# claymore666/openhush

Hardware: AMD Instinct MI355X
Metric: audio-sec/sec (xRT) large-v3 greedy, 30s chunks, 1/2/4/8 MI355X (higher is better)
Workload: dtype bf16; 1 GPU; large-v3 dims, steps of batch=32 x 30 s windows per GPU, greedy, 100 tokens/window (EOT suppressed), procedural weights seed 1234, every window a distinct synthetic recording, PCM resident in HBM; schedule LANES 4x3: 12 steps (384 windows) in flight per GPU - per lane ONE front-end pass and ONE decode batch of 96 rows, 4 decodes side by side on 64 CUs each; concurrent_sub_batches=1

## Files before the change

include/ohw.h:

```cpp
#ifndef OHW_H
#define OHW_H

#include <stddef.h>
#include <stdint.h>

#ifdef __cplusplus
extern "C" {
#endif

#define OHW_ABI_VERSION 2

enum {
  OHW_OK = 0,
  OHW_E_MODEL_NOT_FOUND = -3001,
  OHW_E_LOAD_FAILED = -3002,
  OHW_E_TRANSCRIBE = -3003,
  OHW_E_NO_GPU = -3004,
  OHW_E_OOM = -3005,
  OHW_E_INVALID_ARG = -3006,
  OHW_E_VALIDATION = -3007
};

enum { OHW_DTYPE_AUTO = -1, OHW_DTYPE_BF16 = 0, OHW_DTYPE_F16 = 1 };

// ... 463 lines not shown
typedef struct {
  ohw_dbg_beam_io base;
  const float* plog;
  float* plog_next;
  float* fin_plog;
  float* nosp_prob;
} ohw_dbg_beam_io_ex;
int ohw_dbg_beam_step_ex(ohw_state* st, const ohw_sample_params* p, const ohw_dbg_beam_io_ex* io);

typedef struct {
  int32_t K, W, stride, max_tokens;
  const int32_t* fin_cnt;
  const int32_t* fin_len;
  const float* fin_sum;
  const int32_t* fin_tok;
  const float* fin_plog;
  const int32_t* n_cur;
  const int32_t* tokens;
  const float* plog;
  const float* beam_sum;
  int32_t* out_tokens;
  float* out_logprobs;
  int32_t* n_tokens;
  float* sum_logprob;
  int32_t* ended_by_eot;
  int32_t* n_finished;
} ohw_beam_finish_io;
int ohw_dbg_beam_finish(ohw_state* st, const ohw_beam_finish_io* io);
int ohw_beam_finish_host(const ohw_beam_finish_io* io);

enum { OHW_DEPI_QKV = 0, OHW_DEPI_BIAS_T, OHW_DEPI_BIAS_GELU_T, OHW_DEPI_BIAS_RESID, OHW_DEPI_LOGITS };
enum { OHW_DG_FORM_PLAIN = 0, OHW_DG_FORM_LN, OHW_DG_FORM_PN };
enum { OHW_DG_SHAPE_1x1 = 0, OHW_DG_SHAPE_2x1, OHW_DG_SHAPE_1x2, OHW_DG_SHAPE_2x2, OHW_DG_SHAPE_4x2, OHW_DG_SHAPE_1x6,
       OHW_DG_SHAPE_4x6, OHW_DG_SHAPE_5x6 };
typedef struct {
  int32_t dtype, epilogue, form;
  int32_t M, N, K, n_new;
  int64_t ld_out;
  int32_t cu_budget, ksplit;
  const float* w;
  const float* bias;
  const float* gamma;
  const float* beta;
  const void* x;
  const float* stat_in;
  void* out;
  float* slab;
  int64_t slab_bytes;
  uint32_t* ticket;
  void* x16_out;
  float* stat_out;
  void* k_cache;
  void* v_cache;
  const int32_t* n_past;
  int32_t d_model, n_head, n_ctx;
  int32_t* shape_out;
} ohw_dbg_dec_gemm_io;
int ohw_dbg_dec_gemm(const ohw_dbg_dec_gemm_io* io, void* stream);
int ohw_dbg_embed(int dtype, const float* emb, int n_vocab, const float* pos, int n_pos, const int32_t* tok_host,
                  const int32_t* n_past_host, float* x, void* x16, float* stat, int M, int n_new, int d, void* stream);
int ohw_dbg_layernorm(int dtype, const float* x, const float* gamma, const float* beta, void* y, int64_t rows, int d, int tiled,
                      void* stream);

enum { OHW_EG_KERNEL_AUTO = 0, OHW_EG_KERNEL_K128, OHW_EG_KERNEL_SMALL, OHW_EG_KERNEL_K256 };
typedef struct {
  int32_t dtype, epilogue, kernel;
  int32_t conv_cin;
  int64_t M, N, K;
  int64_t lda, a_batch_stride, rows_per_batch;
  int64_t ldc, c_batch_stride;
  int32_t d_model, n_head, t_len, batch, batch_offset;
  const int32_t* c_row_map;
  const void* a;
  int64_t a_elems;
  const float* w;
  const float* bias;
  const float* pos;
  void* out;
  int64_t out_elems;
} ohw_dbg_enc_gemm_io;
int ohw_dbg_enc_gemm(const ohw_dbg_enc_gemm_io* io, void* stream);

#ifdef __cplusplus
}
#endif
#endif
```

openhush_amd/csrc/decode.hip:

```cpp
#include <algorithm>
#include <type_traits>

#include "kernels.hpp"

namespace ohw {

#ifdef OHW_TRACE
__device__ unsigned long long ohw_trace_buf[1 << 18];
__device__ unsigned ohw_trace_n;
__device__ __forceinline__ void trace_mark(unsigned id, unsigned stage) {
  const unsigned nb = gridDim.x * gridDim.y * gridDim.z, bi = (blockIdx.z * gridDim.y + blockIdx.y) * gridDim.x + blockIdx.x;
  __builtin_amdgcn_sched_barrier(0);
  if (threadIdx.x == 0 && (bi == 0 || bi == nb - 1 || bi == nb / 2)) {
    const unsigned k = atomicAdd(&ohw_trace_n, 1u);
    if (k < (1u << 18)) ohw_trace_buf[k] = ((unsigned long long)wall_clock64() << 16) | (id << 8) | (stage << 2) | (bi == 0 ? 0 : bi == nb - 1 ? 1 : 2);
  }
}
#define TRACE(id, stage) trace_mark(id, stage)
#else
#define TRACE(id, stage)
#endif

template <typename T>
__global__ void embed_kernel(const T* __restrict__ emb, const float* __restrict__ pos, const int32_t* __restrict__ tok,
// ... 493 lines not shown
        else
          self_attn_row<T, false, true>((const T*)p.out, (const T*)p.k_cache, (const T*)p.v_cache, n_keys, m, m, head, p.n_head, p.n_ctx,
                                        nullptr, (T*)p.attn_out, qs, ps, lane, (unsigned)p.kv_bytes);
      }
    }
  }
  TRACE(16 + EPI * 2 + (LN ? 1 : 0), 3);
}

template <typename T, int EPI, bool LN, int NT, int MT>
static int dec_gemm_launch(const DecGemmParams& p, hipStream_t s) {
  const int n_tiles = (p.N + 15) / 16;
  dim3 grid((n_tiles + NT - 1) / NT, (p.M + 16 * MT - 1) / (16 * MT), p.ksplit > 1 ? p.ksplit : 1);
  const size_t smem = (size_t)DG_WAVES * NT * 2 * 64 * 16 + (LN ? (size_t)16 * MT * (p.K * 2 + 16) : 256);
  if (LN) ensure_dynamic_lds((const void*)dec_gemm_kernel<T, EPI, LN, NT, MT>, 160 * 1024);
  hipLaunchKernelGGL((dec_gemm_kernel<T, EPI, LN, NT, MT>), grid, dim3(DG_THREADS), smem, s, p);
  return NT == 4 ? DG_SHAPE_4x2 : NT == 2 ? (MT == 1 ? DG_SHAPE_2x1 : DG_SHAPE_2x2) : (MT == 1 ? DG_SHAPE_1x1 : DG_SHAPE_1x2);
}

template <typename T>
__global__ __launch_bounds__(128) void dec_ln_rows_kernel(const float* __restrict__ x, T* __restrict__ y, int M, int K) {
  const int row = threadIdx.x >> 4, sub = threadIdx.x & 15;
  const int m = blockIdx.x * 8 + row;
  const int mc = m < M ? m : M - 1;
  dec_ln_row<T, 16>(x + (int64_t)mc * K, K, sub, [&](int c, u32x2 w2) {
    if (m >= M) w2 = (u32x2){0u, 0u};
    *(u32x2*)(y + act_tiled_offset(m, c, K)) = w2;
  });
}

template <typename T, int EPI, int NTW, int MTP, int PASSES, int G>
__global__ __launch_bounds__(DG_THREADS, 2) void dec_gemm_rows_kernel(DecGemmParams p) {
  constexpr bool HOLD = EPI != DEPI_BIAS_RESID;
  static_assert(HOLD ? (EPI == DEPI_QKV || EPI == DEPI_BIAS_GELU_T) : (NTW == 1 && PASSES == 1), "rows form");
  using Ops = TypeOps<T>;
  using vec8 = typename Ops::vec8;
  extern __shared__ __attribute__((aligned(16))) unsigned char dg_smem[];
  f32x4* part = (f32x4*)dg_smem;
  const int tid = threadIdx.x, lane = tid & 63, wave = tid >> 6;
  const int nt0 = blockIdx.x * NTW;
  const int n_tiles = (p.N + 15) / 16;
  const int kblocks = p.K / 32;
  TRACE(16 + EPI * 2, 0);
  constexpr int NE = (NTW * MTP * 256 + DG_THREADS - 1) / DG_THREADS;
  [[maybe_unused]] float resid_old[NE];
  if constexpr (!HOLD) {
#pragma unroll
    for (int i = 0; i < NE; ++i) {
      const int idx = tid + DG_THREADS * i, ll = (idx >> 2) & 63;
      const int m = (blockIdx.y * MTP + (idx >> 8)) * 16 + (ll & 15), n = nt0 * 16 + 4 * (ll >> 4) + (idx & 3);
      resid_old[i] = (idx < MTP * 256 && m < p.M && n < p.N) ? ((const float*)p.out)[(int64_t)m * p.ld_out + n] : 0.f;
    }
  }
  const vec8* wt[NTW];
#pragma unroll
  for (int t = 0; t < NTW; ++t) {
    int nt = nt0 + t;
    if (nt > n_tiles - 1) nt = n_tiles - 1;
    wt[t] = (const vec8*)p.w + (int64_t)nt * kblocks * 64 + lane;
  }
  constexpr int UL = DG_LN_MAXK / 32 / DG_WAVES;
  [[maybe_unused]] vec8 whold[HOLD ? NTW : 1][UL];
  if constexpr (HOLD) {
#pragma unroll
    for (int u = 0; u < UL; ++u) {
      int kk = wave + DG_WAVES * u;
      if (kk > kblocks - 1) kk = kblocks - 1;
#pragma unroll
      for (int t = 0; t < NTW; ++t) whold[t][u] = __builtin_nontemporal_load(&wt[t][(int64_t)kk * 64]);
    }
  }

#pragma unroll 1
  for (int pass = 0; pass < PASSES; ++pass) {
    const int mt0 = (blockIdx.y * PASSES + pass) * MTP;
    if (mt0 * 16 >= p.M) break;
    [[maybe_unused]] const T* x0 = (const T*)p.x + ((int64_t)mt0 * kblocks * 64 + lane) * 8;
    bool ok[MTP];
#pragma unroll
    for (int q = 0; q < MTP; ++q) ok[q] = (mt0 + q) * 16 + (lane & 15) < p.M;
    f32x4 acc[NTW][MTP];
#pragma unroll
    for (int t = 0; t < NTW; ++t)
#pragma unroll
      for (int q = 0; q < MTP; ++q) acc[t][q] = (f32x4){0.f, 0.f, 0.f, 0.f};

    if constexpr (HOLD) {
      typedef __attribute__((ext_vector_type(4))) unsigned u32v4;
      const int mt_last = (p.M - 1) >> 4;
      u32v4 a32[MTP][UL];
#pragma unroll
      for (int q = 0; q < MTP; ++q) {
        const int mq = mt0 + q < mt_last ? mt0 + q : mt_last;
        const T* xq = (const T*)p.x + ((int64_t)mq * kblocks * 64 + lane) * 8;
#pragma unroll
        for (int u = 0; u < UL; ++u) {
          const int kk = wave + DG_WAVES * u;
          a32[q][u] = *(const u32v4*)(xq + (int64_t)(kk < kblocks ? kk : 0) * 512);
        }
      }
      vec8 a[MTP][UL];
#pragma unroll
      for (int q = 0; q < MTP; ++q)
#pragma unroll
        for (int u = 0; u < UL; ++u) {
          const unsigned keep = (ok[q] && wave + DG_WAVES * u < kblocks) ? 0xffffffffu : 0u;
          a[q][u] = __builtin_bit_cast(vec8, a32[q][u] & keep);
        }
      __builtin_amdgcn_sched_barrier(0);
#pragma unroll
      for (int u = 0; u < UL; ++u)
#pragma unroll
        for (int t = 0; t < NTW; ++t)
#pragma unroll
          for (int q = 0; q < MTP; ++q) acc[t][q] = Ops::mfma16(whold[t][u], a[q][u], acc[t][q]);
    } else {
      auto run = [&](auto ucount, int kb) {
        constexpr int U = decltype(ucount)::value;
        constexpr int GG = U < G ? U : G;
        static_assert(U % GG == 0, "U");
        vec8 w[U];
#pragma unroll
        for (int u = 0; u < U; ++u) w[u] = __builtin_nontemporal_load(&wt[0][(int64_t)(kb + DG_WAVES * u) * 64]);
#pragma unroll
        for (int g = 0; g < U; g += GG) {
          vec8 a[MTP][GG];
#pragma unroll
          for (int q = 0; q < MTP; ++q) {
#pragma unroll
            for (int u = 0; u < GG; ++u)
#pragma unroll
// ... 10 lines not shown
            for (int q = 0; q < MTP; ++q) acc[0][q] = Ops::mfma16(w[g + u], a[q][u], acc[0][q]);
        }
      };
      int kb = wave;
      for (; kb + DG_WAVES * 19 < kblocks; kb += DG_WAVES * 20) run(std::integral_constant<int, 20>{}, kb);
      for (; kb + DG_WAVES * 3 < kblocks; kb += DG_WAVES * 4) run(std::integral_constant<int, 4>{}, kb);
      for (; kb < kblocks; kb += DG_WAVES) run(std::integral_constant<int, 1>{}, kb);
    }

    TRACE(16 + EPI * 2, 2);
    int etid = tid;
    if constexpr (HOLD) {
      __builtin_amdgcn_sched_barrier(0);
      asm volatile("" : "+v"(etid));
    }
    if (pass > 0) __syncthreads();
#pragma unroll
    for (int t = 0; t < NTW; ++t)
#pragma unroll
      for (int q = 0; q < MTP; ++q) part[((wave * NTW + t) * MTP + q) * 64 + lane] = acc[t][q];
    __syncthreads();
    const float* pp = (const float*)part;
#pragma unroll
    for (int i = 0; i < NE; ++i) {
      const int idx = etid + DG_THREADS * i;
      if (idx >= NTW * MTP * 256) continue;
      const int t = idx / (MTP * 256), q = (idx % (MTP * 256)) >> 8, ll = (idx >> 2) & 63, reg = idx & 3;
      float v = 0.f;
#pragma unroll
      for (int w = 0; w < DG_WAVES; ++w) v += pp[(((w * NTW + t) * MTP + q) * 64 + ll) * 4 + reg];
      const int m = (mt0 + q) * 16 + (ll & 15), n = (nt0 + t) * 16 + 4 * (ll >> 4) + reg;
      if (m >= p.M || n >= p.N || nt0 + t >= n_tiles) continue;
      if (p.bias) v += p.bias[n];
      if constexpr (HOLD) dec_gemm_store16<T, EPI>(p, m, n, v);
      else ((float*)p.out)[(int64_t)m * p.ld_out + n] = resid_old[i] + v;
    }
  }
  TRACE(16 + EPI * 2, 3);
}

template <typename T, int EPI, int NTW, int MTP, int PASSES, int G>
static void dec_gemm_rows_launch(const DecGemmParams& p, hipStream_t s) {
  const int n_tiles = (p.N + 15) / 16, mt = (p.M + 15) / 16;
  const size_t smem = (size_t)DG_WAVES * NTW * MTP * 64 * 16;
  if (smem > 64 * 1024) ensure_dynamic_lds((const void*)dec_gemm_rows_kernel<T, EPI, NTW, MTP, PASSES, G>, 160 * 1024);
  hipLaunchKernelGGL((dec_gemm_rows_kernel<T, EPI, NTW, MTP, PASSES, G>), dim3((n_tiles + NTW - 1) / NTW, (mt + MTP * PASSES - 1) / (MTP * PASSES)),
                     dim3(DG_THREADS), smem, s, p);
}

template <typename T, int EPI, int NTW>
static int dec_gemm_lnrows_launch(const DecGemmParams& p, hipStream_t s) {
  const int mt = (p.M + 15) / 16;
  hipLaunchKernelGGL((dec_ln_rows_kernel<T>), dim3(2 * mt), dim3(128), 0, s, (const float*)p.x, (T*)p.ln_rows, p.M, p.K);
  DecGemmParams q = p;
  q.x = p.ln_rows; q.ln = 0;
  dec_gemm_rows_launch<T, EPI, NTW, 3, 2, 5>(q, s);
  return NTW == 4 ? DG_SHAPE_4x6 : DG_SHAPE_5x6;
}

template <typename T, int EPI, bool LN>
static int dec_gemm_pick(const DecGemmParams& p, hipStream_t s) {
  const int n_tiles = (p.N + 15) / 16;
  static const int logits_nt = getenv("OHW_LOGITS_NT") ? atoi(getenv("OHW_LOGITS_NT")) : 2;
  static const int msplit = getenv("OHW_DEC_MSPLIT") ? atoi(getenv("OHW_DEC_MSPLIT")) : 1;
  const int cus = p.cu_budget > 0 ? p.cu_budget : 256;
  const int mt = (p.M + 15) / 16;
  if constexpr (EPI == DEPI_BIAS_RESID && !LN) {
    if (msplit && p.ksplit <= 1 && (mt == 1 || n_tiles * mt <= 2 * cus)) return dec_gemm_launch<T, EPI, LN, 1, 1>(p, s);
  }
  if constexpr (!LN && (EPI == DEPI_QKV || EPI == DEPI_BIAS_T || EPI == DEPI_BIAS_GELU_T)) {
    if (p.pn && msplit && mt <= 2) {
      if (n_tiles * mt <= cus) return dec_gemm_launch<T, EPI, LN, 1, 1>(p, s);
      if ((n_tiles + 1) / 2 * mt <= cus || mt == 1) return dec_gemm_launch<T, EPI, LN, 2, 1>(p, s);
    }
    if (p.pn && n_tiles > cus) return dec_gemm_launch<T, EPI, LN, 2, 2>(p, s);
  }
  if constexpr (LN) {
    if (msplit && mt <= 2) {
      if (n_tiles * mt <= cus) return dec_gemm_launch<T, EPI, LN, 1, 1>(p, s);
      if ((n_tiles + 1) / 2 * mt <= cus || mt == 1) return dec_gemm_launch<T, EPI, LN, 2, 1>(p, s);
    }
  }
  if constexpr (EPI == DEPI_LOGITS) {
    if (msplit && mt == 1 && logits_nt == 2) return dec_gemm_launch<T, EPI, LN, 2, 1>(p, s);
  }
  if constexpr (LN && (EPI == DEPI_QKV || EPI == DEPI_BIAS_GELU_T)) {
    static const int lnrows = getenv("OHW_DEC_LNROWS") ? atoi(getenv("OHW_DEC_LNROWS")) : 1;
    if (lnrows && p.ln_rows && mt > 2 && p.K <= DG_LN_MAXK && !p.pn && p.ksplit <= 1 && !p.stat_out && !p.attn_ticket &&
        (int64_t)((n_tiles + 3) / 4) * ((mt + 1) / 2) > 2 * cus) {
      if (EPI == DEPI_BIAS_GELU_T && (n_tiles + 3) / 4 > cus) {
        if ((n_tiles + 4) / 5 >= 32) return dec_gemm_lnrows_launch<T, EPI, 5>(p, s);
      } else if ((n_tiles + 3) / 4 >= 32) {
        return dec_gemm_lnrows_launch<T, EPI, 4>(p, s);
      }
    }
  }
  static const int nt4 = getenv("OHW_DEC_NT4") ? atoi(getenv("OHW_DEC_NT4")) : 1;
  if constexpr ((LN && (EPI == DEPI_QKV || EPI == DEPI_BIAS_T || EPI == DEPI_BIAS_GELU_T)) || (!LN && (EPI == DEPI_BIAS_RESID || EPI == DEPI_LOGITS))) {
    const int64_t wgs = LN ? (int64_t)((n_tiles + 1) / 2) * ((mt + 1) / 2) : (int64_t)n_tiles * ((mt + 1) / 2);
    if (nt4 && mt > 2 && p.ksplit <= 1 && !p.pn && !p.stat_out && p.K <= DG_LN_MAXK && wgs > 2 * cus) return dec_gemm_launch<T, EPI, LN, 4, 2>(p, s);
  }
  if constexpr (EPI == DEPI_BIAS_RESID && !LN) {
    static const int rows = getenv("OHW_DEC_ROWS") ? atoi(getenv("OHW_DEC_ROWS")) : 1;
    if (rows && mt > 2 && p.ksplit <= 1 && !p.pn && !p.stat_out && p.K > DG_LN_MAXK && (int64_t)n_tiles * ((mt + 1) / 2) > 2 * cus)
    {
      dec_gemm_rows_launch<T, DEPI_BIAS_RESID, 1, 6, 1, 4>(p, s);
      return DG_SHAPE_1x6;
    }
  }
  if ((LN && n_tiles > cus) || (EPI == DEPI_LOGITS && logits_nt == 2)) return dec_gemm_launch<T, EPI, LN, 2, 2>(p, s);
  return dec_gemm_launch<T, EPI, LN, 1, 2>(p, s);
}

template <typename T>
int launch_dec_gemm(const DecGemmParams& p, int epilogue, hipStream_t s) {
  if (p.K % 32 != 0) throw Error(OHW_E_INVALID_ARG, "dec_gemm: K must be a multiple of 32");
  const bool ln = p.ln != 0;
  if (p.ksplit > 1) {
    const int64_t tiles = (int64_t)((p.N + 15) / 16) * ((p.M + 31) / 32);
    if (epilogue != DEPI_BIAS_RESID || !p.slab || !p.ticket || tiles * p.ksplit * 2048 > p.slab_bytes || p.ksplit > p.K / 32)
      throw Error(OHW_E_INVALID_ARG, "dec_gemm: split-K needs the RESID epilogue and a slab of tiles * ksplit * 2 KiB");
  }
  if (ln && (p.K % 64 != 0 || p.K > DG_LN_MAXK)) throw Error(OHW_E_INVALID_ARG, "dec_gemm: fused LayerNorm needs K <= 1280, K % 64 == 0");
  if (p.pn && (ln || !p.stat_in || !p.wsum || p.n_stat * 16 != p.K || p.n_stat > 128)) throw Error(OHW_E_INVALID_ARG, "dec_gemm: post-norm needs statistics of K / 16 tiles per row and the weights' row sums");
  if (p.stat_out && (epilogue != DEPI_BIAS_RESID || !p.x16_out || p.N % 32 != 0 || p.ksplit > 1))
    throw Error(OHW_E_INVALID_ARG, "dec_gemm: statistics come from the unsplit RESID epilogue with N % 32 == 0");
  if (epilogue == DEPI_BIAS_GELU_T && p.N % 32 != 0) throw Error(OHW_E_INVALID_ARG, "dec_gemm: the tiled GELU output needs N % 32 == 0");
  int shape = 0;
// ... 1550 lines not shown
```

openhush_amd/csrc/engine.hip:

```cpp
#include <execinfo.h>
#include <signal.h>
#include <unistd.h>

#include <cstring>
#include <memory>
#include <mutex>
#include <shared_mutex>
#include <type_traits>
#include <vector>
#include <algorithm>

#include "attention.hpp"
#include "dequant.hpp"
#include "gemm.hpp"
#include "kernels.hpp"
#include "model.hpp"

namespace ohw {
ohw_ctx* ctx_from_file(const char* path, int device, int dtype);
ohw_ctx* ctx_synthetic(const ohw_hparams* hp, uint32_t seed, int device, int dtype);
ohw_ctx* ctx_shell(const ohw_hparams* hp, int device, int dtype);
void select_device(int device);

thread_local std::string g_last_error;
// ... 34 lines not shown
  } catch (const Error& e) {
    g_last_error = e.what();
    return e.code;
  } catch (const std::bad_alloc&) {
    g_last_error = "host allocation failed";
    return OHW_E_OOM;
  } catch (const std::exception& e) {
    g_last_error = e.what();
    return OHW_E_TRANSCRIBE;
  } catch (...) {
    g_last_error = "unknown error";
    return OHW_E_TRANSCRIBE;
  }
}
}

using namespace ohw;

constexpr int DEC_KSPLIT_MAX = 8;
static int env_int(const char* name, int dflt, int lo, int hi) {
  const char* e = getenv(name);
  if (!e || !*e) return dflt;
  const int v = atoi(e);
  return v < lo ? lo : v > hi ? hi : v;
}
static int dec_ksplit_long() { return env_int("OHW_DEC_KSPLIT_LONG", 1, 1, DEC_KSPLIT_MAX); }
static int dec_ksplit_short() { return env_int("OHW_DEC_KSPLIT_SHORT", 1, 1, DEC_KSPLIT_MAX); }


enum DecTallyGemm { DT_QKV, DT_O, DT_XQ, DT_XO, DT_FC1, DT_FC2, DT_LOGITS, DT_GEMMS };
enum DecTallyForm { DT_PLAIN, DT_LN, DT_PN, DT_KSPLIT, DT_FORMS };
static const char* const kDecTallyGemm[DT_GEMMS] = {"qkv", "o", "xq", "xo", "fc1", "fc2", "logits"};
static const char* const kDecTallyForm[DT_FORMS] = {"", ".ln", ".pn", ".ks"};
static const char* const kDecTallyShape[DG_N_SHAPES] = {"1x1", "2x1", "1x2", "2x2", "4x2", "1x6", "4x6", "5x6"};
static const char* const kXattnTally[XA_N_VARIANTS] = {"plain", "split", "rows2", "rows3", "rows4", "group2", "group3", "group4", "group5", "group_split"};
static const char* const kSelfAttnTally[4] = {"plain", "slots", "fused", "fused_slots"};

#define BMARK(what, i) do { static const bool on_ = env_int("OHW_DEBUG_MARKS", 0, 0, 1) != 0; if (on_) { std::fprintf(stderr, "[ohw beam] %s %d\n", what, (int)(i)); std::fflush(stderr); } } while (0)

struct GraphKey {
  int rows = 0;
  int group = 0;
  int cus = 0;
  int t_len = 0;
  bool var = false, invariant = false, persist = false;
  bool flag = false;
  bool phrases = false;
  SamplerParams spar;
  bool operator==(const GraphKey& o) const {
    return rows == o.rows && group == o.group && cus == o.cus && t_len == o.t_len && var == o.var && invariant == o.invariant &&
           persist == o.persist && flag == o.flag && phrases == o.phrases && std::memcmp(&spar, &o.spar, sizeof spar) == 0;
  }
};
struct GraphEntry {
  GraphKey key;
  hipGraph_t graph[2] = {nullptr, nullptr};
  hipGraphExec_t exec[2] = {nullptr, nullptr};
  void destroy() {
    for (int q = 0; q < 2; ++q) {
      if (exec[q]) (void)hipGraphExecDestroy(exec[q]);
      if (graph[q]) (void)hipGraphDestroy(graph[q]);
    }
  }
};
struct GraphCache {
  size_t capacity;
  bool marks = false;
// ... 2862 lines not shown
                      int n_new, int n_head, int n_ctx, const int32_t* kv_slot_host, int* variant_out, void* stream) {
  return guard([&] {
    dbg_check_dtype(dtype, "dbg_self_attn");
    if (!q || !k_cache || !v_cache || !n_past_host || !out || M < 1 || n_new < 1 || n_head < 1 || n_ctx < 1)
      throw Error(OHW_E_INVALID_ARG, "dbg_self_attn: null buffer, or M, n_new, n_head or n_ctx below 1");
    if (M % n_new != 0) throw Error(OHW_E_INVALID_ARG, "dbg_self_attn: M must be a multiple of n_new");
    const int rows = M / n_new;
    for (int b = 0; b < rows; ++b)
      if (n_past_host[b] < 0 || (int64_t)n_past_host[b] + n_new > n_ctx)
        throw Error(OHW_E_INVALID_ARG, "dbg_self_attn: n_past[" + std::to_string(b) + "] = " + std::to_string(n_past_host[b]) + " with n_new = " + std::to_string(n_new) +
                                           " is outside the " + std::to_string(n_ctx) + " positions of the cache");
    for (int64_t i = 0; kv_slot_host && i < (int64_t)rows * n_ctx; ++i)
      if (kv_slot_host[i] < 0 || kv_slot_host[i] >= rows)
        throw Error(OHW_E_INVALID_ARG, "dbg_self_attn: kv_slot[" + std::to_string(i / n_ctx) + "][" + std::to_string(i % n_ctx) + "] = " + std::to_string(kv_slot_host[i]) +
                                           " names no cache row (0 .. " + std::to_string(rows - 1) + ")");
    DevBuf past, slots;
    dbg_upload(past, n_past_host, (size_t)rows);
    if (kv_slot_host) dbg_upload(slots, kv_slot_host, (size_t)rows * n_ctx);
    int variant = -1;
    Dispatch::run(dtype, [&](auto* tag) {
      using TT = std::remove_pointer_t<decltype(tag)>;
      variant = launch_self_attn<TT>(q, k_cache, v_cache, past.as<int32_t>(), out, M, n_new, n_head, n_ctx, (hipStream_t)stream,
                                     kv_slot_host ? slots.as<int32_t>() : nullptr);
    });
    HIP_CHECK(hipStreamSynchronize((hipStream_t)stream));
    if (variant_out) *variant_out = variant;
  });
}

static_assert(OHW_DEPI_QKV == DEPI_QKV && OHW_DEPI_BIAS_T == DEPI_BIAS_T && OHW_DEPI_BIAS_GELU_T == DEPI_BIAS_GELU_T &&
              OHW_DEPI_BIAS_RESID == DEPI_BIAS_RESID && OHW_DEPI_LOGITS == DEPI_LOGITS, "ohw.h names kernels.hpp's epilogues");
static_assert(OHW_DG_SHAPE_1x1 == DG_SHAPE_1x1 && OHW_DG_SHAPE_2x1 == DG_SHAPE_2x1 && OHW_DG_SHAPE_1x2 == DG_SHAPE_1x2 &&
              OHW_DG_SHAPE_2x2 == DG_SHAPE_2x2 && OHW_DG_SHAPE_4x2 == DG_SHAPE_4x2 && OHW_DG_SHAPE_1x6 == DG_SHAPE_1x6 &&
              OHW_DG_SHAPE_4x6 == DG_SHAPE_4x6 && OHW_DG_SHAPE_5x6 == DG_SHAPE_5x6, "ohw.h names kernels.hpp's shapes");

int ohw_dbg_dec_gemm(const ohw_dbg_dec_gemm_io* io, void* stream) {
  return guard([&] {
    if (!io) throw Error(OHW_E_INVALID_ARG, "dbg_dec_gemm: null io");
    const ohw_dbg_dec_gemm_io& a = *io;
    auto bad = [](const std::string& why) { throw Error(OHW_E_INVALID_ARG, "dbg_dec_gemm: " + why); };
    dbg_check_dtype(a.dtype, "dbg_dec_gemm");
    if (a.epilogue < DEPI_QKV || a.epilogue > DEPI_LOGITS) bad("epilogue must be 0 .. 4");
    if (a.form < OHW_DG_FORM_PLAIN || a.form > OHW_DG_FORM_PN) bad("form must be 0 (plain), 1 (ln) or 2 (pn)");
    if (!a.w || !a.x || !a.out) bad("null w, x or out");
    if (a.M < 1 || a.N < 1 || a.K < 32 || a.M > (1 << 20) || a.N > (1 << 20) || a.K > (1 << 20)) bad("M, N >= 1 and K >= 32 (each at most 2^20)");
    if (a.K % 32 != 0) bad("K = " + std::to_string(a.K) + " must be a multiple of 32");
    if (a.cu_budget < 0 || a.ksplit < 0) bad("cu_budget and ksplit must not be negative");
    if ((a.gamma == nullptr) != (a.beta == nullptr)) bad("gamma and beta come together");
    const bool ln = a.form == OHW_DG_FORM_LN, pn = a.form == OHW_DG_FORM_PN;
    const bool t_epi = a.epilogue == DEPI_QKV || a.epilogue == DEPI_BIAS_T || a.epilogue == DEPI_BIAS_GELU_T;
    if ((ln || pn) && !t_epi) bad("the ln and pn forms exist for the QKV, BIAS_T and BIAS_GELU_T epilogues");
    if (ln && a.K > 1280) bad("ln: K = " + std::to_string(a.K) + " exceeds the 1280 columns of the fused LayerNorm");
    if (ln && a.K % 64 != 0) bad("ln: K = " + std::to_string(a.K) + " must be a multiple of 64");
    if (pn && a.K / 16 > 128) bad("pn: n_stat = K / 16 = " + std::to_string(a.K / 16) + " exceeds 128 statistics tiles per row");
    if (pn && !a.stat_in) bad("pn: null stat_in");
    const bool uses_ld = a.epilogue == DEPI_BIAS_T || a.epilogue == DEPI_BIAS_RESID || a.epilogue == DEPI_LOGITS;
    if (uses_ld && a.ld_out < a.N) bad("ld_out = " + std::to_string(a.ld_out) + " is below N = " + std::to_string(a.N));
    if (a.epilogue == DEPI_BIAS_GELU_T && a.N % 32 != 0) bad("BIAS_GELU_T writes activation tiles: N = " + std::to_string(a.N) + " must be a multiple of 32");
    const bool rows_epi = a.epilogue == DEPI_QKV || a.epilogue == DEPI_LOGITS;
    if (rows_epi && (a.n_new < 1 || a.M % a.n_new != 0)) bad("M = " + std::to_string(a.M) + " must be a multiple of n_new = " + std::to_string(a.n_new) + " >= 1");
    const int windows = rows_epi ? a.M / a.n_new : 0;
    if (a.epilogue == DEPI_QKV) {
      if (!a.k_cache || !a.v_cache || !a.n_past) bad("QKV: null k_cache, v_cache or n_past");
      if (a.n_head < 1 || a.n_ctx < 1 || a.d_model != 64 * a.n_head || a.N != 3 * a.d_model) bad("QKV: d_model == 64 * n_head, N == 3 * d_model, n_ctx >= 1");
      for (int b = 0; b < windows; ++b)
        if (a.n_past[b] < 0 || a.n_past[b] > a.n_ctx)
          bad("n_past[" + std::to_string(b) + "] = " + std::to_string(a.n_past[b]) + " is outside 0 .. n_ctx = " + std::to_string(a.n_ctx));
// ... 7 lines not shown
        bad("split-K: slab_bytes = " + std::to_string(a.slab_bytes) + ", needed " + std::to_string(tiles * a.ksplit * 2048) + " (tiles * ksplit * 2 KiB, below 2 GiB)");
    }
    if ((a.x16_out == nullptr) != (a.stat_out == nullptr)) bad("x16_out and stat_out come together");
    if (a.stat_out) {
      if (a.epilogue != DEPI_BIAS_RESID || a.ksplit > 1) bad("stat_out: statistics come from the unsplit RESID epilogue");
      if (a.N % 32 != 0) bad("stat_out: N = " + std::to_string(a.N) + " must be a multiple of 32");
    }

    hipStream_t s = (hipStream_t)stream;
    const int64_t n_pad = ((int64_t)a.N + 15) / 16 * 16;
    DevBuf wf, bf, wt, ws, past, lnr;
    wf.alloc((size_t)a.N * a.K * 4);
    HIP_CHECK(hipMemcpyAsync(wf.p, a.w, (size_t)a.N * a.K * 4, hipMemcpyDeviceToDevice, s));
    const bool own_bias = a.bias != nullptr || a.gamma != nullptr;
    if (own_bias) {
      bf.alloc((size_t)a.N * 4);
      if (a.bias) HIP_CHECK(hipMemcpyAsync(bf.p, a.bias, (size_t)a.N * 4, hipMemcpyDeviceToDevice, s));
      else HIP_CHECK(hipMemsetAsync(bf.p, 0, (size_t)a.N * 4, s));
    }
    if (a.gamma) launch_fold_ln(wf.as<float>(), bf.as<float>(), a.gamma, a.beta, a.N, a.K, s);
    wt.alloc((size_t)n_pad * a.K * 2);
    if (pn) ws.alloc((size_t)a.N * 4);
    if (ln) lnr.alloc(((size_t)a.M + 15) / 16 * 16 * a.K * 2);
    if (a.epilogue == DEPI_QKV) dbg_upload(past, a.n_past, (size_t)windows);
    int shape = -1;
    Dispatch::run(a.dtype, [&](auto* tag) {
      using TT = std::remove_pointer_t<decltype(tag)>;
      launch_repack_tiled<TT>(wf.as<float>(), wt.p, a.N, n_pad, a.K, s);
      if (pn) launch_tiled_rowsum<TT>(wt.p, ws.as<float>(), a.N, a.K, s);
      DecGemmParams p{};
      p.x = a.x; p.ln = ln ? 1 : 0; p.ln_rows = lnr.p; p.w = wt.p; p.bias = own_bias ? bf.as<float>() : nullptr; p.out = a.out;
      p.M = a.M; p.N = a.N; p.K = a.K; p.n_new = rows_epi ? a.n_new : 1;
      p.ld_out = a.epilogue == DEPI_QKV ? a.d_model : a.ld_out; p.cu_budget = a.cu_budget;
      if (a.epilogue == DEPI_QKV) {
        p.k_cache = a.k_cache; p.v_cache = a.v_cache; p.n_past = past.as<int32_t>();
        p.d_model = a.d_model; p.n_head = a.n_head; p.n_ctx = a.n_ctx;
      }
      if (a.ksplit > 1) { p.ksplit = a.ksplit; p.slab = a.slab; p.slab_bytes = (int32_t)a.slab_bytes; p.ticket = a.ticket; }
      if (pn) { p.pn = 1; p.n_stat = a.K / 16; p.stat_in = a.stat_in; p.wsum = ws.as<float>(); }
      if (a.stat_out) { p.x16_out = a.x16_out; p.stat_out = a.stat_out; }
      shape = launch_dec_gemm<TT>(p, a.epilogue, s);
    });
    HIP_CHECK(hipStreamSynchronize(s));
    if (a.shape_out) *a.shape_out = shape;
  });
}

int ohw_dbg_embed(int dtype, const float* emb, int n_vocab, const float* pos, int n_pos, const int32_t* tok_host,
                  const int32_t* n_past_host, float* x, void* x16, float* stat, int M, int n_new, int d, void* stream) {
  return guard([&] {
    dbg_check_dtype(dtype, "dbg_embed");
    if (!emb || !pos || !tok_host || !n_past_host || !x || n_vocab < 1 || n_pos < 1 || M < 1 || n_new < 1 || d < 32)
      throw Error(OHW_E_INVALID_ARG, "dbg_embed: null buffer, or n_vocab, n_pos, M or n_new below 1, or d below 32");
    if (d % 32 != 0 || d > (1 << 16) || n_vocab > (1 << 20)) throw Error(OHW_E_INVALID_ARG, "dbg_embed: d must be a multiple of 32 (at most 2^16), n_vocab at most 2^20");
    if (M % n_new != 0) throw Error(OHW_E_INVALID_ARG, "dbg_embed: M must be a multiple of n_new");
    for (int m = 0; m < M; ++m)
      if (tok_host[m] < 0 || tok_host[m] >= n_vocab)
        throw Error(OHW_E_INVALID_ARG, "dbg_embed: tok[" + std::to_string(m) + "] = " + std::to_string(tok_host[m]) + " is outside the " + std::to_string(n_vocab) + " rows of the table");
    for (int b = 0; b < M / n_new; ++b)
      if (n_past_host[b] < 0 || (int64_t)n_past_host[b] + n_new > n_pos)
        throw Error(OHW_E_INVALID_ARG, "dbg_embed: n_past[" + std::to_string(b) + "] = " + std::to_string(n_past_host[b]) + " with n_new = " + std::to_string(n_new) +
                                           " is outside the " + std::to_string(n_pos) + " positions");
    hipStream_t s = (hipStream_t)stream;
    const int64_t v_pad = ((int64_t)n_vocab + 15) / 16 * 16;
    DevBuf et, tok, past;
    et.alloc((size_t)v_pad * d * 2);
// ... 112 lines not shown
```

openhush_amd/csrc/kernels.hpp:

```cpp
#pragma once
#include <vector>

#include "common.hpp"

namespace ohw {

void launch_synth_fill(float* dst, int64_t n, uint32_t key, float scale, float offset, int round_f16, hipStream_t s);
void launch_f16_to_f32(const void* src_f16, float* dst, int64_t n, hipStream_t s);
void launch_dequant_blocks(int ttype, const void* raw_blocks, float* dst, int64_t n, hipStream_t s);
template <typename T> void launch_convert_rows(const float* src, void* dst, int64_t rows, int64_t cols, int64_t ld_dst, hipStream_t s);
template <typename T> void launch_repack_conv(const float* src, void* dst, int64_t d_out, int64_t c_in, int64_t c_pad, hipStream_t s);
template <typename T> void launch_repack_tiled(const float* src, void* dst, int64_t N, int64_t n_pad, int64_t K, hipStream_t s);
template <typename T> void launch_tiled_rowsum(const void* w_tiled, float* wsum, int64_t N, int64_t K, hipStream_t s);
void launch_fold_ln(float* w, float* bias, const float* gamma, const float* beta, int64_t N, int64_t K, hipStream_t s);

struct MelParams {
  const float* pcm;
  int64_t pcm_stride;
  const int32_t* n_samples;
  const float* filters;
  const float* twiddle;
  const float* window;
  float* logmel;
  int32_t* max_bits;
// ... 20 lines not shown
  DEPI_QKV = 0,
  DEPI_BIAS_T = 1,
  DEPI_BIAS_GELU_T = 2,
  DEPI_BIAS_RESID = 3,
  DEPI_LOGITS = 4
};
struct DecGemmParams {
  const void* x;
  int32_t ln;
  const void* w;
  const float* bias;
  void* out;
  int32_t M, N, K, n_new;
  void* k_cache; void* v_cache;
  const int32_t* n_past;
  int32_t d_model, n_head, n_ctx;
  int64_t ld_out;
  int32_t cu_budget;
  int32_t ksplit;
  int32_t slab_bytes;
  float* slab;
  unsigned* ticket;
  int32_t pn;
  int32_t n_stat;
  const float* stat_in;
  const float* wsum;
  void* x16_out;
  float* stat_out;
  unsigned* attn_ticket;
  void* attn_out;
  const int32_t* attn_slots;
  int64_t kv_bytes;
  void* ln_rows;
};
enum DecGemmShape { DG_SHAPE_1x1, DG_SHAPE_2x1, DG_SHAPE_1x2, DG_SHAPE_2x2, DG_SHAPE_4x2, DG_SHAPE_1x6, DG_SHAPE_4x6, DG_SHAPE_5x6, DG_N_SHAPES };
template <typename T> int launch_dec_gemm(const DecGemmParams& p, int epilogue, hipStream_t s);

template <typename T> void launch_embed(const void* emb_tiled, const float* pos, const int32_t* tok, const int32_t* n_past,
                                        float* x, void* x16, float* stat, int M, int n_new, int d, hipStream_t s);
enum SelfAttnVariant { SA_PLAIN, SA_SLOTS };
template <typename T> int launch_self_attn(const void* q, const void* k_cache, const void* v_cache, const int32_t* n_past,
                                            void* out, int M, int n_new, int n_head, int n_ctx, hipStream_t s, const int32_t* kv_slot = nullptr);
constexpr int XA_MAX_SPLIT = 8;
enum XattnVariant { XA_PLAIN, XA_SPLIT, XA_ROWS2, XA_ROWS3, XA_ROWS4, XA_GROUP2, XA_GROUP3, XA_GROUP4, XA_GROUP5, XA_GROUP_SPLIT, XA_N_VARIANTS };
template <typename T> int launch_cross_attn(const void* q, const void* xk, const void* xv, void* out, int M, int n_new,
                                             int n_head, int t_len, float* partials, unsigned* tickets, int max_split_rows,
                                             const int32_t* done , hipStream_t s,
                                             int kv_group = 1 ,
                                             bool batch_invariant = false ,
                                             const int32_t* win_len = nullptr );
template <typename T> void launch_cross_attn_chunk(const void* q, const void* xk, const void* xv, void* out, int windows, int n_head, int t_len,
                                                   const int32_t* done, const int32_t* win_len, hipStream_t s, int n_q = 8);

struct PersistLayer {
  const void *wqkv, *wo, *wxq, *wxo, *w1, *w2;
  const float *bqkv, *bo, *bxq, *bxo, *b1, *b2;
};
struct PersistParams {
  const PersistLayer* layers;
  int32_t L, M, group, d, H, n_ctx, t_len, S, nsplit;
  const int32_t* n_past;
  const int32_t* kv_slot;
  const int32_t* done;
  const float* x_in;
  float* x_out;
  void* self_kv;
  int64_t kv_layer, kv_row;
  const void* xkv;
// ... 159 lines not shown
```

openhush_amd/engine.py:

```python
from __future__ import annotations

import ctypes as C
import dataclasses
import os
import time
from typing import List, Optional, Sequence, Tuple, Union

import numpy as np

_HERE = os.path.dirname(os.path.abspath(__file__))
LIB_PATH = os.environ.get("OHW_LIB") or os.path.join(_HERE, "libohw.so")

CHUNK_SAMPLES = 480000
CHUNK_FRAMES = 3000

OHW_DTYPE_AUTO, OHW_DTYPE_BF16, OHW_DTYPE_F16 = -1, 0, 1
OHW_MEL_REFLECT, OHW_MEL_ZERO_TAIL = 0, 1
OHW_WINDOW_FIXED, OHW_WINDOW_SEEK, OHW_WINDOW_FIXED_RECORDING_MEL = 0, 1, 2
OHW_SCHEDULE_SEQUENTIAL, OHW_SCHEDULE_PIPELINE, OHW_SCHEDULE_LANES = 0, 1, 2
EPI_BIAS_T, EPI_BIAS_GELU_T, EPI_BIAS_RESID_F32, EPI_F32 = 0, 1, 2, 4
XA_PLAIN, XA_SPLIT, XA_ROWS2, XA_ROWS3, XA_ROWS4, XA_GROUP2, XA_GROUP3, XA_GROUP4, XA_GROUP5, XA_GROUP_SPLIT = range(10)
SA_PLAIN, SA_SLOTS = 0, 1

OHW_E_MODEL_NOT_FOUND, OHW_E_LOAD_FAILED, OHW_E_TRANSCRIBE = -3001, -3002, -3003
# ... 65 lines not shown


class DbgBeamIO(C.Structure):
    _fields_ = ([(n, C.c_int32) for n in ("first", "K", "W", "side")] + [("logits", C.POINTER(C.c_float))] +
                [(n, C.POINTER(C.c_float) if n in ("beam_sum", "fin_sum", "cand_lp") else C.POINTER(C.c_int32))
                 for n in ("tokens", "kv_slot", "n_cur", "n_past_w", "win_done", "beam_sum", "fin_cnt", "fin_tok", "fin_len", "fin_sum",
                           "cand_tok", "cand_lp", "tokens_next", "kv_slot_next", "next_tok", "n_past", "n_done")] +
                [("tickets_out", C.POINTER(C.c_uint32))])


class BeamResultEx(C.Structure):
    _fields_ = [("tokens", C.POINTER(C.c_int32)), ("n_tokens", C.POINTER(C.c_int32)), ("sum_logprob", C.POINTER(C.c_float)),
                ("n_finished", C.POINTER(C.c_int32)), ("token_logprobs", C.POINTER(C.c_float)), ("ended_by_eot", C.POINTER(C.c_int32)),
                ("no_speech_prob", C.POINTER(C.c_float))]


class DbgBeamIOEx(C.Structure):
    _fields_ = [("base", DbgBeamIO), ("plog", C.POINTER(C.c_float)), ("plog_next", C.POINTER(C.c_float)), ("fin_plog", C.POINTER(C.c_float)),
                ("nosp_prob", C.POINTER(C.c_float))]


class BeamFinishIO(C.Structure):
    _fields_ = ([(n, C.c_int32) for n in ("K", "W", "stride", "max_tokens")] +
                [(n, C.POINTER(C.c_float) if n in ("fin_sum", "fin_plog", "plog", "beam_sum", "out_logprobs", "sum_logprob") else C.POINTER(C.c_int32))
                 for n in ("fin_cnt", "fin_len", "fin_sum", "fin_tok", "fin_plog", "n_cur", "tokens", "plog", "beam_sum", "out_tokens",
                           "out_logprobs", "n_tokens", "sum_logprob", "ended_by_eot", "n_finished")])


class DbgDecGemmIO(C.Structure):
    _fields_ = ([(n, C.c_int32) for n in ("dtype", "epilogue", "form", "M", "N", "K", "n_new")] + [("ld_out", C.c_int64)] +
                [(n, C.c_int32) for n in ("cu_budget", "ksplit")] +
                [(n, C.c_void_p) for n in ("w", "bias", "gamma", "beta", "x", "stat_in", "out", "slab")] + [("slab_bytes", C.c_int64)] +
                [(n, C.c_void_p) for n in ("ticket", "x16_out", "stat_out", "k_cache", "v_cache")] + [("n_past", C.POINTER(C.c_int32))] +
                [(n, C.c_int32) for n in ("d_model", "n_head", "n_ctx")] + [("shape_out", C.POINTER(C.c_int32))])


class DbgEncGemmIO(C.Structure):
    _fields_ = ([(n, C.c_int32) for n in ("dtype", "epilogue", "kernel", "conv_cin")] +
                [(n, C.c_int64) for n in ("M", "N", "K", "lda", "a_batch_stride", "rows_per_batch", "ldc", "c_batch_stride")] +
                [(n, C.c_int32) for n in ("d_model", "n_head", "t_len", "batch", "batch_offset")] + [("c_row_map", C.POINTER(C.c_int32))] +
                [("a", C.c_void_p), ("a_elems", C.c_int64), ("w", C.c_void_p), ("bias", C.c_void_p), ("pos", C.c_void_p), ("out", C.c_void_p),
                 ("out_elems", C.c_int64)])


EPI_GELU_POS_F32, EPI_CROSSKV_T = 3, 5
EG_KERNEL_AUTO, EG_KERNEL_K128, EG_KERNEL_SMALL, EG_KERNEL_K256 = range(4)

DEPI_QKV, DEPI_BIAS_T, DEPI_BIAS_GELU_T, DEPI_BIAS_RESID, DEPI_LOGITS = range(5)
DG_FORM_PLAIN, DG_FORM_LN, DG_FORM_PN = range(3)
DG_SHAPE_1x1, DG_SHAPE_2x1, DG_SHAPE_1x2, DG_SHAPE_2x2, DG_SHAPE_4x2, DG_SHAPE_1x6, DG_SHAPE_4x6, DG_SHAPE_5x6 = range(8)

OHW_DBG_SENTINEL_I32 = -7777777
OHW_DBG_SENTINEL_F32 = -12345.0


def _beam_finish(handle, K: int, state: dict, max_tokens: Optional[int]) -> dict:
    W = int(np.asarray(state["n_cur"]).size)
    R = W * K
    S = int(np.asarray(state["tokens"]).shape[1])
    n = S if max_tokens is None else int(max_tokens)
    i32 = lambda k, shape: np.array(state[k], dtype=np.int32, order="C").reshape(shape)
    f32 = lambda k, shape: np.array(state[k], dtype=np.float32, order="C").reshape(shape)
    a = dict(fin_cnt=i32("fin_cnt", W), fin_len=i32("fin_len", R), fin_sum=f32("fin_sum", R), fin_tok=i32("fin_tok", (R, S)),
             fin_plog=f32("fin_plog", (R, S + 1)), n_cur=i32("n_cur", W), tokens=i32("tokens", (R, S)), plog=f32("plog", (R, S + 1)),
             beam_sum=f32("beam_sum", R), out_tokens=np.zeros((W, max(n, 0)), np.int32), out_logprobs=np.zeros((W, max(n, 0) + 1), np.float32),
             n_tokens=np.zeros(W, np.int32), sum_logprob=np.zeros(W, np.float32), ended_by_eot=np.zeros(W, np.int32),
             n_finished=np.zeros(W, np.int32))
    io = BeamFinishIO(K, W, S, n, *[(_fp(a[k]) if a[k].dtype == np.float32 else _ip(a[k])) for k, _ in BeamFinishIO._fields_[4:]])
    _check(lib().ohw_beam_finish_host(C.byref(io)) if handle is None else lib().ohw_dbg_beam_finish(handle, C.byref(io)))
    return {"tokens": a["out_tokens"], "logprobs": a["out_logprobs"], "n_tokens": a["n_tokens"], "sum_logprob": a["sum_logprob"],
            "ended_by_eot": a["ended_by_eot"], "n_finished": a["n_finished"]}


def beam_finish_host(K: int, state: dict, max_tokens: Optional[int] = None) -> dict:
    return _beam_finish(None, K, state, max_tokens)


PHRASE_MAX_LEN, PHRASE_MAX_PHRASES = 16, 1024
PHRASE_MAX_NODES = 1 + PHRASE_MAX_PHRASES * (PHRASE_MAX_LEN - 1)
PHRASE_MAX_EDGES = PHRASE_MAX_PHRASES * PHRASE_MAX_LEN
PHRASE_MAX_PATH = PHRASE_MAX_PHRASES * (PHRASE_MAX_LEN - 1) * PHRASE_MAX_LEN // 2


# ... 2204 lines not shown
```

Baseline: 4105 audio-sec/sec.

## Add weight-holding rows kernel for logits and NT4 tiling for LN cross-query GEMM

```diff
diff --git a/include/ohw.h b/include/ohw.h
--- a/include/ohw.h
+++ b/include/ohw.h
@@ -519,7 +519,7 @@
 enum { OHW_DEPI_QKV = 0, OHW_DEPI_BIAS_T, OHW_DEPI_BIAS_GELU_T, OHW_DEPI_BIAS_RESID, OHW_DEPI_LOGITS };
 enum { OHW_DG_FORM_PLAIN = 0, OHW_DG_FORM_LN, OHW_DG_FORM_PN };
 enum { OHW_DG_SHAPE_1x1 = 0, OHW_DG_SHAPE_2x1, OHW_DG_SHAPE_1x2, OHW_DG_SHAPE_2x2, OHW_DG_SHAPE_4x2, OHW_DG_SHAPE_1x6,
-       OHW_DG_SHAPE_4x6, OHW_DG_SHAPE_5x6 };
+       OHW_DG_SHAPE_4x6, OHW_DG_SHAPE_5x6, OHW_DG_SHAPE_4x6P };
 typedef struct {
   int32_t dtype, epilogue, form;
   int32_t M, N, K, n_new;
@@ -542,6 +542,7 @@
   const int32_t* n_past;
   int32_t d_model, n_head, n_ctx;
   int32_t* shape_out;
+  int32_t tail_forms_off;
 } ohw_dbg_dec_gemm_io;
 int ohw_dbg_dec_gemm(const ohw_dbg_dec_gemm_io* io, void* stream);
 int ohw_dbg_embed(int dtype, const float* emb, int n_vocab, const float* pos, int n_pos, const int32_t* tok_host,
diff --git a/openhush_amd/csrc/decode.hip b/openhush_amd/csrc/decode.hip
--- a/openhush_amd/csrc/decode.hip
+++ b/openhush_amd/csrc/decode.hip
@@ -549,7 +549,8 @@
 template <typename T, int EPI, int NTW, int MTP, int PASSES, int G>
 __global__ __launch_bounds__(DG_THREADS, 2) void dec_gemm_rows_kernel(DecGemmParams p) {
   constexpr bool HOLD = EPI != DEPI_BIAS_RESID;
-  static_assert(HOLD ? (EPI == DEPI_QKV || EPI == DEPI_BIAS_GELU_T) : (NTW == 1 && PASSES == 1), "rows form");
+  constexpr bool LNR = EPI == DEPI_QKV || EPI == DEPI_BIAS_GELU_T;
+  static_assert(HOLD ? (LNR || EPI == DEPI_LOGITS) : (NTW == 1 && PASSES == 1), "rows form");
   using Ops = TypeOps<T>;
   using vec8 = typename Ops::vec8;
   extern __shared__ __attribute__((aligned(16))) unsigned char dg_smem[];
@@ -610,10 +611,22 @@
       for (int q = 0; q < MTP; ++q) {
         const int mq = mt0 + q < mt_last ? mt0 + q : mt_last;
         const T* xq = (const T*)p.x + ((int64_t)mq * kblocks * 64 + lane) * 8;
-#pragma unroll
-        for (int u = 0; u < UL; ++u) {
-          const int kk = wave + DG_WAVES * u;
-          a32[q][u] = *(const u32v4*)(xq + (int64_t)(kk < kblocks ? kk : 0) * 512);
+        if constexpr (LNR) {
+#pragma unroll
+          for (int u = 0; u < UL; ++u) {
+            const int kk = wave + DG_WAVES * u;
+            a32[q][u] = *(const u32v4*)(xq + (int64_t)(kk < kblocks ? kk : 0) * 512);
+          }
+        } else {
+#pragma unroll
+          for (int u = 0; u < UL; ++u) a32[q][u] = (u32v4){0u, 0u, 0u, 0u};
+          if (ok[q]) {
+#pragma unroll
+            for (int u = 0; u < UL; ++u) {
+              const int kk = wave + DG_WAVES * u;
+              a32[q][u] = *(const u32v4*)(xq + (int64_t)(kk < kblocks ? kk : 0) * 512);
+            }
+          }
         }
       }
       vec8 a[MTP][UL];
@@ -690,8 +703,13 @@
       const int m = (mt0 + q) * 16 + (ll & 15), n = (nt0 + t) * 16 + 4 * (ll >> 4) + reg;
       if (m >= p.M || n >= p.N || nt0 + t >= n_tiles) continue;
       if (p.bias) v += p.bias[n];
-      if constexpr (HOLD) dec_gemm_store16<T, EPI>(p, m, n, v);
-      else ((float*)p.out)[(int64_t)m * p.ld_out + n] = resid_old[i] + v;
+      if constexpr (EPI == DEPI_LOGITS) {
+        if (m % p.n_new == p.n_new - 1) ((float*)p.out)[(int64_t)(m / p.n_new) * p.ld_out + n] = v;
+      } else if constexpr (HOLD) {
+        dec_gemm_store16<T, EPI>(p, m, n, v);
+      } else {
+        ((float*)p.out)[(int64_t)m * p.ld_out + n] = resid_old[i] + v;
+      }
     }
   }
   TRACE(16 + EPI * 2, 3);
@@ -752,6 +770,20 @@
         return dec_gemm_lnrows_launch<T, EPI, 4>(p, s);
       }
     }
+  }
+  if constexpr (EPI == DEPI_LOGITS && !LN) {
+    static const int lrows = getenv("OHW_DEC_LOGITS_ROWS") ? atoi(getenv("OHW_DEC_LOGITS_ROWS")) : 1;
+    if (lrows && !p.tail_forms_off && p.cu_budget >= 32 && mt > 2 && p.K <= DG_LN_MAXK && p.ksplit <= 1 && !p.pn && !p.stat_out &&
+        (int64_t)n_tiles * ((mt + 1) / 2) > 2 * cus && (n_tiles + 3) / 4 >= 8) {
+      dec_gemm_rows_launch<T, DEPI_LOGITS, 4, 3, 2, 5>(p, s);
+      return DG_SHAPE_4x6P;
+    }
+  }
+  if constexpr (LN && EPI == DEPI_BIAS_T) {
+    static const int xq4 = getenv("OHW_DEC_XQ_NT4") ? atoi(getenv("OHW_DEC_XQ_NT4")) : 1;
+    const int64_t g2 = (int64_t)((n_tiles + 1) / 2) * ((mt + 1) / 2), g4 = (int64_t)((n_tiles + 3) / 4) * ((mt + 1) / 2);
+    if (xq4 && !p.tail_forms_off && p.cu_budget > 0 && mt > 2 && p.K <= DG_LN_MAXK && g2 > cus && g4 <= cus && g4 >= 32)
+      return dec_gemm_launch<T, EPI, LN, 4, 2>(p, s);
   }
   static const int nt4 = getenv("OHW_DEC_NT4") ? atoi(getenv("OHW_DEC_NT4")) : 1;
   if constexpr ((LN && (EPI == DEPI_QKV || EPI == DEPI_BIAS_T || EPI == DEPI_BIAS_GELU_T)) || (!LN && (EPI == DEPI_BIAS_RESID || EPI == DEPI_LOGITS))) {
diff --git a/openhush_amd/csrc/engine.hip b/openhush_amd/csrc/engine.hip
--- a/openhush_amd/csrc/engine.hip
+++ b/openhush_amd/csrc/engine.hip
@@ -90,7 +90,7 @@
 enum DecTallyForm { DT_PLAIN, DT_LN, DT_PN, DT_KSPLIT, DT_FORMS };
 static const char* const kDecTallyGemm[DT_GEMMS] = {"qkv", "o", "xq", "xo", "fc1", "fc2", "logits"};
 static const char* const kDecTallyForm[DT_FORMS] = {"", ".ln", ".pn", ".ks"};
-static const char* const kDecTallyShape[DG_N_SHAPES] = {"1x1", "2x1", "1x2", "2x2", "4x2", "1x6", "4x6", "5x6"};
+static const char* const kDecTallyShape[DG_N_SHAPES] = {"1x1", "2x1", "1x2", "2x2", "4x2", "1x6", "4x6", "5x6", "4x6p"};
 static const char* const kXattnTally[XA_N_VARIANTS] = {"plain", "split", "rows2", "rows3", "rows4", "group2", "group3", "group4", "group5", "group_split"};
 static const char* const kSelfAttnTally[4] = {"plain", "slots", "fused", "fused_slots"};
 
@@ -3019,7 +3019,7 @@
               OHW_DEPI_BIAS_RESID == DEPI_BIAS_RESID && OHW_DEPI_LOGITS == DEPI_LOGITS, "ohw.h names kernels.hpp's epilogues");
 static_assert(OHW_DG_SHAPE_1x1 == DG_SHAPE_1x1 && OHW_DG_SHAPE_2x1 == DG_SHAPE_2x1 && OHW_DG_SHAPE_1x2 == DG_SHAPE_1x2 &&
               OHW_DG_SHAPE_2x2 == DG_SHAPE_2x2 && OHW_DG_SHAPE_4x2 == DG_SHAPE_4x2 && OHW_DG_SHAPE_1x6 == DG_SHAPE_1x6 &&
-              OHW_DG_SHAPE_4x6 == DG_SHAPE_4x6 && OHW_DG_SHAPE_5x6 == DG_SHAPE_5x6, "ohw.h names kernels.hpp's shapes");
+              OHW_DG_SHAPE_4x6 == DG_SHAPE_4x6 && OHW_DG_SHAPE_5x6 == DG_SHAPE_5x6 && OHW_DG_SHAPE_4x6P == DG_SHAPE_4x6P, "ohw.h names kernels.hpp's shapes");
 
 int ohw_dbg_dec_gemm(const ohw_dbg_dec_gemm_io* io, void* stream) {
   return guard([&] {
@@ -3093,6 +3093,7 @@
       p.x = a.x; p.ln = ln ? 1 : 0; p.ln_rows = lnr.p; p.w = wt.p; p.bias = own_bias ? bf.as<float>() : nullptr; p.out = a.out;
       p.M = a.M; p.N = a.N; p.K = a.K; p.n_new = rows_epi ? a.n_new : 1;
       p.ld_out = a.epilogue == DEPI_QKV ? a.d_model : a.ld_out; p.cu_budget = a.cu_budget;
+      p.tail_forms_off = a.tail_forms_off;
       if (a.epilogue == DEPI_QKV) {
         p.k_cache = a.k_cache; p.v_cache = a.v_cache; p.n_past = past.as<int32_t>();
         p.d_model = a.d_model; p.n_head = a.n_head; p.n_ctx = a.n_ctx;
diff --git a/openhush_amd/csrc/kernels.hpp b/openhush_amd/csrc/kernels.hpp
--- a/openhush_amd/csrc/kernels.hpp
+++ b/openhush_amd/csrc/kernels.hpp
@@ -76,8 +76,10 @@
   const int32_t* attn_slots;
   int64_t kv_bytes;
   void* ln_rows;
-};
-enum DecGemmShape { DG_SHAPE_1x1, DG_SHAPE_2x1, DG_SHAPE_1x2, DG_SHAPE_2x2, DG_SHAPE_4x2, DG_SHAPE_1x6, DG_SHAPE_4x6, DG_SHAPE_5x6, DG_N_SHAPES };
+  int32_t tail_forms_off;
+};
+enum DecGemmShape { DG_SHAPE_1x1, DG_SHAPE_2x1, DG_SHAPE_1x2, DG_SHAPE_2x2, DG_SHAPE_4x2, DG_SHAPE_1x6, DG_SHAPE_4x6, DG_SHAPE_5x6, DG_SHAPE_4x6P,
+                    DG_N_SHAPES };
 template <typename T> int launch_dec_gemm(const DecGemmParams& p, int epilogue, hipStream_t s);
 
 template <typename T> void launch_embed(const void* emb_tiled, const float* pos, const int32_t* tok, const int32_t* n_past,
diff --git a/openhush_amd/engine.py b/openhush_amd/engine.py
--- a/openhush_amd/engine.py
+++ b/openhush_amd/engine.py
@@ -121,7 +121,7 @@
                 [(n, C.c_int32) for n in ("cu_budget", "ksplit")] +
                 [(n, C.c_void_p) for n in ("w", "bias", "gamma", "beta", "x", "stat_in", "out", "slab")] + [("slab_bytes", C.c_int64)] +
                 [(n, C.c_void_p) for n in ("ticket", "x16_out", "stat_out", "k_cache", "v_cache")] + [("n_past", C.POINTER(C.c_int32))] +
-                [(n, C.c_int32) for n in ("d_model", "n_head", "n_ctx")] + [("shape_out", C.POINTER(C.c_int32))])
+                [(n, C.c_int32) for n in ("d_model", "n_head", "n_ctx")] + [("shape_out", C.POINTER(C.c_int32)), ("tail_forms_off", C.c_int32)])
 
 
 class DbgEncGemmIO(C.Structure):
@@ -137,7 +137,7 @@
 
 DEPI_QKV, DEPI_BIAS_T, DEPI_BIAS_GELU_T, DEPI_BIAS_RESID, DEPI_LOGITS = range(5)
 DG_FORM_PLAIN, DG_FORM_LN, DG_FORM_PN = range(3)
-DG_SHAPE_1x1, DG_SHAPE_2x1, DG_SHAPE_1x2, DG_SHAPE_2x2, DG_SHAPE_4x2, DG_SHAPE_1x6, DG_SHAPE_4x6, DG_SHAPE_5x6 = range(8)
+DG_SHAPE_1x1, DG_SHAPE_2x1, DG_SHAPE_1x2, DG_SHAPE_2x2, DG_SHAPE_4x2, DG_SHAPE_1x6, DG_SHAPE_4x6, DG_SHAPE_5x6, DG_SHAPE_4x6P = range(9)
 
 OHW_DBG_SENTINEL_I32 = -7777777
 OHW_DBG_SENTINEL_F32 = -12345.0
```

After: 3996 audio-sec/sec. 2.7% lower.
